# neonbjb/tortoise-tts

Hardware: NVIDIA H100
Metric: audio-seconds/sec at preset='standard' (higher is better)
Workload: dtype bf16 tensor-core operands, fp32 accumulate/residual/norm/softmax/scheduler

## Files before the change

tortoise_tts_b200/csrc/common.cuh:

```cuda
#pragma once
#include <cuda_runtime.h>
#include <cuda_bf16.h>
#include <cuda.h>
#include <stdint.h>
#include <cstdlib>

#define TTB_DEVINL __device__ __forceinline__

namespace ttb {

void set_error(const char* fmt, ...);
int check_cuda(cudaError_t e, const char* what);
#define TTB_CHECK_LAUNCH(what)                                   \
  do {                                                           \
    cudaError_t _e = cudaGetLastError();                         \
    if (_e != cudaSuccess) return ttb::check_cuda(_e, what);     \
  } while (0)

TTB_DEVINL void pdl_wait() { asm volatile("griddepcontrol.wait;" ::: "memory"); }
TTB_DEVINL void pdl_launch_dependents() { asm volatile("griddepcontrol.launch_dependents;" ::: "memory"); }

inline bool pdl_enabled() {
  static int v = -1;
  if (v < 0) {
    const char* e = getenv("TTB_PDL");
    v = (e && e[0] == '0') ? 0 : 1;
  }
  return v == 1;
}

template <typename... KArgs, typename... Args>
inline cudaError_t launch_pdl(void (*kernel)(KArgs...), dim3 grid, dim3 block, size_t smem, cudaStream_t st, Args&&... args) {
  cudaLaunchConfig_t cfg = {};
  cfg.gridDim = grid;
  cfg.blockDim = block;
  cfg.dynamicSmemBytes = smem;
  cfg.stream = st;
  cudaLaunchAttribute at[1];
  if (pdl_enabled()) {
    at[0].id = cudaLaunchAttributeProgrammaticStreamSerialization;
    at[0].val.programmaticStreamSerializationAllowed = 1;
    cfg.attrs = at;
    cfg.numAttrs = 1;
  }
  return cudaLaunchKernelEx(&cfg, kernel, static_cast<KArgs>(args)...);
}

TTB_DEVINL float silu(float x) { return x / (1.0f + __expf(-x)); }
TTB_DEVINL float gelu_new(float x) {
  const float k = 0.7978845608028654f;
  float u = k * (x + 0.044715f * x * x * x);
  return 0.5f * x * (1.0f + tanhf(u));
}
TTB_DEVINL float gelu_erf(float x) { return 0.5f * x * (1.0f + erff(x * 0.7071067811865476f)); }
TTB_DEVINL float leaky(float x, float s) { return x > 0.f ? x : x * s; }

TTB_DEVINL float warp_sum(float v) {
#pragma unroll
  for (int o = 16; o > 0; o >>= 1) v += __shfl_xor_sync(0xffffffffu, v, o);
  return v;
}
TTB_DEVINL float warp_max(float v) {
#pragma unroll
  for (int o = 16; o > 0; o >>= 1) v = fmaxf(v, __shfl_xor_sync(0xffffffffu, v, o));
  return v;
}

TTB_DEVINL float block_sum(float v, float* red) {
  int lane = threadIdx.x & 31, w = threadIdx.x >> 5, nw = (blockDim.x + 31) >> 5;
  v = warp_sum(v);
  __syncthreads();
  if (lane == 0) red[w] = v;
  __syncthreads();
  float r = (lane < nw) ? red[lane] : 0.f;
  r = warp_sum(r);
  return r;
}
TTB_DEVINL float block_max(float v, float* red) {
  int lane = threadIdx.x & 31, w = threadIdx.x >> 5, nw = (blockDim.x + 31) >> 5;
  v = warp_max(v);
  __syncthreads();
  if (lane == 0) red[w] = v;
  __syncthreads();
  float r = (lane < nw) ? red[lane] : -INFINITY;
  r = warp_max(r);
  return r;
}

TTB_DEVINL uint32_t pack_bf16(float a, float b) {
  __nv_bfloat162 t = __floats2bfloat162_rn(a, b);
  return *reinterpret_cast<uint32_t*>(&t);
}
TTB_DEVINL float2 unpack_bf16(uint32_t u) {
  __nv_bfloat162 t = *reinterpret_cast<__nv_bfloat162*>(&u);
  return __bfloat1622float2(t);
}

TTB_DEVINL uint32_t smem_u32(const void* p) { return static_cast<uint32_t>(__cvta_generic_to_shared(p)); }

TTB_DEVINL unsigned long long global_timer_ns() {
  unsigned long long t;
  asm volatile("mov.u64 %0, %%globaltimer;" : "=l"(t));
  return t;
}
TTB_DEVINL unsigned long long sm_id() {
  uint32_t s;
  asm volatile("mov.u32 %0, %%smid;" : "=r"(s));
  return s;
}

TTB_DEVINL bool elect_one() {
  uint32_t pred = 0;
  asm volatile(
      "{\n\t.reg .pred P;\n\t.reg .b32 R;\n\t"
      "elect.sync R|P, 0xffffffff;\n\t"
      "selp.u32 %0, 1, 0, P;\n\t}\n"
      : "=r"(pred));
  return pred != 0;
}

TTB_DEVINL void mbar_init(uint64_t* bar, uint32_t count) {
  asm volatile("mbarrier.init.shared::cta.b64 [%0], %1;" ::"r"(smem_u32(bar)), "r"(count));
}
TTB_DEVINL void fence_barrier_init() { asm volatile("fence.mbarrier_init.release.cluster;" ::: "memory"); }
TTB_DEVINL void fence_proxy_async() { asm volatile("fence.proxy.async.shared::cta;" ::: "memory"); }
TTB_DEVINL void mbar_arrive_expect_tx(uint64_t* bar, uint32_t bytes) {
  asm volatile("mbarrier.arrive.expect_tx.shared::cta.b64 _, [%0], %1;" ::"r"(smem_u32(bar)), "r"(bytes) : "memory");
}
TTB_DEVINL void mbar_arrive(uint64_t* bar) {
  asm volatile("mbarrier.arrive.shared::cta.b64 _, [%0];" ::"r"(smem_u32(bar)) : "memory");
}
#ifndef TTB_MBAR_HINT_NS
#define TTB_MBAR_HINT_NS 20000
#endif
TTB_DEVINL void mbar_wait(uint64_t* bar, uint32_t parity) {
#if TTB_MBAR_HINT_NS > 0
  asm volatile(
      "{\n\t.reg .pred P1;\n\t"
      "WAIT_LOOP:\n\t"
      "mbarrier.try_wait.parity.shared::cta.b64 P1, [%0], %1, %2;\n\t"
      "@P1 bra DONE;\n\t"
      "bra WAIT_LOOP;\n\t"
      "DONE:\n\t}\n" ::"r"(smem_u32(bar)),
      "r"(parity), "r"((uint32_t)TTB_MBAR_HINT_NS)
      : "memory");
#else
  asm volatile(
      "{\n\t.reg .pred P1;\n\t"
      "WAIT_LOOP:\n\t"
      "mbarrier.try_wait.parity.shared::cta.b64 P1, [%0], %1;\n\t"
      "@P1 bra DONE;\n\t"
      "bra WAIT_LOOP;\n\t"
      "DONE:\n\t}\n" ::"r"(smem_u32(bar)),
      "r"(parity)
      : "memory");
#endif
}

TTB_DEVINL void tma_prefetch_desc(const CUtensorMap* m) {
  asm volatile("prefetch.tensormap [%0];" ::"l"(reinterpret_cast<uint64_t>(m)) : "memory");
}
TTB_DEVINL void tma_load_2d(void* smem_dst, const CUtensorMap* map, uint64_t* bar, int c0, int c1) {
  asm volatile(
      "cp.async.bulk.tensor.2d.shared::cluster.global.mbarrier::complete_tx::bytes [%0], [%1, {%3, %4}], [%2];"
      ::"r"(smem_u32(smem_dst)), "l"(reinterpret_cast<uint64_t>(map)), "r"(smem_u32(bar)), "r"(c0), "r"(c1)
      : "memory");
}
TTB_DEVINL void tma_load_3d(void* smem_dst, const CUtensorMap* map, uint64_t* bar, int c0, int c1, int c2) {
  asm volatile(
      "cp.async.bulk.tensor.3d.shared::cluster.global.mbarrier::complete_tx::bytes [%0], [%1, {%3, %4, %5}], [%2];"
      ::"r"(smem_u32(smem_dst)), "l"(reinterpret_cast<uint64_t>(map)), "r"(smem_u32(bar)), "r"(c0), "r"(c1), "r"(c2)
      : "memory");
}
TTB_DEVINL void tma_prefetch_l2_3d(const CUtensorMap* map, int c0, int c1, int c2) {
  asm volatile("cp.async.bulk.prefetch.tensor.3d.L2.global.tile [%0, {%1, %2, %3}];"
               ::"l"(reinterpret_cast<uint64_t>(map)), "r"(c0), "r"(c1), "r"(c2)
               : "memory");
}

TTB_DEVINL void wgmma_fence() { asm volatile("wgmma.fence.sync.aligned;" ::: "memory"); }
TTB_DEVINL void wgmma_commit() { asm volatile("wgmma.commit_group.sync.aligned;" ::: "memory"); }
template <int N>
TTB_DEVINL void wgmma_wait() { asm volatile("wgmma.wait_group.sync.aligned %0;" ::"n"(N) : "memory"); }
TTB_DEVINL void named_barrier(int id, int nthreads) { asm volatile("bar.sync %0, %1;" ::"r"(id), "r"(nthreads) : "memory"); }

TTB_DEVINL uint64_t wgmma_desc_kmajor_sw128(uint32_t smem_addr) {
  uint64_t d = 0;
  d |= (uint64_t)((smem_addr & 0x3FFFF) >> 4);
  d |= (uint64_t)1 << 16;
  d |= (uint64_t)(1024 >> 4) << 32;
  d |= (uint64_t)1 << 62;
  return d;
}
TTB_DEVINL uint64_t wgmma_desc_mnmajor_sw128(uint32_t smem_addr, uint32_t lbo_bytes) {
  uint64_t d = 0;
  d |= (uint64_t)((smem_addr & 0x3FFFF) >> 4);
  d |= (uint64_t)((lbo_bytes >> 4) & 0x3FFF) << 16;
  d |= (uint64_t)(1024 >> 4) << 32;
  d |= (uint64_t)1 << 62;
  return d;
}

TTB_DEVINL void wgmma_m64n16k16_bf16_ss(float* d, uint64_t desc_a, uint64_t desc_b, uint32_t scale_d) {
  asm volatile(
      "{\n\t.reg .pred p;\n\tsetp.ne.b32 p, %10, 0;\n\t"
      "wgmma.mma_async.sync.aligned.m64n16k16.f32.bf16.bf16 {%0, %1, %2, %3, %4, %5, %6, %7}, %8, %9, p, 1, 1, 0, 0;\n\t}\n"
      : "+f"(d[0]), "+f"(d[1]), "+f"(d[2]), "+f"(d[3]), "+f"(d[4]), "+f"(d[5]), "+f"(d[6]), "+f"(d[7])
      : "l"(desc_a), "l"(desc_b), "r"(scale_d));
}
TTB_DEVINL void wgmma_m64n32k16_bf16_ss(float* d, uint64_t desc_a, uint64_t desc_b, uint32_t scale_d) {
  asm volatile(
      "{\n\t.reg .pred p;\n\tsetp.ne.b32 p, %18, 0;\n\t"
      "wgmma.mma_async.sync.aligned.m64n32k16.f32.bf16.bf16 {%0, %1, %2, %3, %4, %5, %6, %7, %8, %9, %10, %11, %12, %13, %14, %15}, %16, %17, p, 1, 1, 0, 0;\n\t}\n"
      : "+f"(d[0]), "+f"(d[1]), "+f"(d[2]), "+f"(d[3]), "+f"(d[4]), "+f"(d[5]), "+f"(d[6]), "+f"(d[7]), "+f"(d[8]), "+f"(d[9]), "+f"(d[10]), "+f"(d[11]), "+f"(d[12]), "+f"(d[13]), "+f"(d[14]), "+f"(d[15])
      : "l"(desc_a), "l"(desc_b), "r"(scale_d));
}
TTB_DEVINL void wgmma_m64n64k16_bf16_ss(float* d, uint64_t desc_a, uint64_t desc_b, uint32_t scale_d) {
  asm volatile(
      "{\n\t.reg .pred p;\n\tsetp.ne.b32 p, %34, 0;\n\t"
      "wgmma.mma_async.sync.aligned.m64n64k16.f32.bf16.bf16 {%0, %1, %2, %3, %4, %5, %6, %7, %8, %9, %10, %11, %12, %13, %14, %15, %16, %17, %18, %19, %20, %21, %22, %23, %24, %25, %26, %27, %28, %29, %30, %31}, %32, %33, p, 1, 1, 0, 0;\n\t}\n"
      : "+f"(d[0]), "+f"(d[1]), "+f"(d[2]), "+f"(d[3]), "+f"(d[4]), "+f"(d[5]), "+f"(d[6]), "+f"(d[7]), "+f"(d[8]), "+f"(d[9]), "+f"(d[10]), "+f"(d[11]), "+f"(d[12]), "+f"(d[13]), "+f"(d[14]), "+f"(d[15]), "+f"(d[16]), "+f"(d[17]), "+f"(d[18]), "+f"(d[19]), "+f"(d[20]), "+f"(d[21]), "+f"(d[22]), "+f"(d[23]), "+f"(d[24]), "+f"(d[25]), "+f"(d[26]), "+f"(d[27]), "+f"(d[28]), "+f"(d[29]), "+f"(d[30]), "+f"(d[31])
      : "l"(desc_a), "l"(desc_b), "r"(scale_d));
}
TTB_DEVINL void wgmma_m64n256k16_bf16_ss(float* d, uint64_t desc_a, uint64_t desc_b, uint32_t scale_d) {
  asm volatile(
      "{\n\t.reg .pred p;\n\tsetp.ne.b32 p, %130, 0;\n\t"
      "wgmma.mma_async.sync.aligned.m64n256k16.f32.bf16.bf16 {%0, %1, %2, %3, %4, %5, %6, %7, %8, %9, %10, %11, %12, %13, %14, %15, %16, %17, %18, %19, %20, %21, %22, %23, %24, %25, %26, %27, %28, %29, %30, %31, %32, %33, %34, %35, %36, %37, %38, %39, %40, %41, %42, %43, %44, %45, %46, %47, %48, %49, %50, %51, %52, %53, %54, %55, %56, %57, %58, %59, %60, %61, %62, %63, %64, %65, %66, %67, %68, %69, %70, %71, %72, %73, %74, %75, %76, %77, %78, %79, %80, %81, %82, %83, %84, %85, %86, %87, %88, %89, %90, %91, %92, %93, %94, %95, %96, %97, %98, %99, %100, %101, %102, %103, %104, %105, %106, %107, %108, %109, %110, %111, %112, %113, %114, %115, %116, %117, %118, %119, %120, %121, %122, %123, %124, %125, %126, %127}, %128, %129, p, 1, 1, 0, 0;\n\t}\n"
      : "+f"(d[0]), "+f"(d[1]), "+f"(d[2]), "+f"(d[3]), "+f"(d[4]), "+f"(d[5]), "+f"(d[6]), "+f"(d[7]), "+f"(d[8]), "+f"(d[9]), "+f"(d[10]), "+f"(d[11]), "+f"(d[12]), "+f"(d[13]), "+f"(d[14]), "+f"(d[15]), "+f"(d[16]), "+f"(d[17]), "+f"(d[18]), "+f"(d[19]), "+f"(d[20]), "+f"(d[21]), "+f"(d[22]), "+f"(d[23]), "+f"(d[24]), "+f"(d[25]), "+f"(d[26]), "+f"(d[27]), "+f"(d[28]), "+f"(d[29]), "+f"(d[30]), "+f"(d[31]), "+f"(d[32]), "+f"(d[33]), "+f"(d[34]), "+f"(d[35]), "+f"(d[36]), "+f"(d[37]), "+f"(d[38]), "+f"(d[39]), "+f"(d[40]), "+f"(d[41]), "+f"(d[42]), "+f"(d[43]), "+f"(d[44]), "+f"(d[45]), "+f"(d[46]), "+f"(d[47]), "+f"(d[48]), "+f"(d[49]), "+f"(d[50]), "+f"(d[51]), "+f"(d[52]), "+f"(d[53]), "+f"(d[54]), "+f"(d[55]), "+f"(d[56]), "+f"(d[57]), "+f"(d[58]), "+f"(d[59]), "+f"(d[60]), "+f"(d[61]), "+f"(d[62]), "+f"(d[63]), "+f"(d[64]), "+f"(d[65]), "+f"(d[66]), "+f"(d[67]), "+f"(d[68]), "+f"(d[69]), "+f"(d[70]), "+f"(d[71]), "+f"(d[72]), "+f"(d[73]), "+f"(d[74]), "+f"(d[75]), "+f"(d[76]), "+f"(d[77]), "+f"(d[78]), "+f"(d[79]), "+f"(d[80]), "+f"(d[81]), "+f"(d[82]), "+f"(d[83]), "+f"(d[84]), "+f"(d[85]), "+f"(d[86]), "+f"(d[87]), "+f"(d[88]), "+f"(d[89]), "+f"(d[90]), "+f"(d[91]), "+f"(d[92]), "+f"(d[93]), "+f"(d[94]), "+f"(d[95]), "+f"(d[96]), "+f"(d[97]), "+f"(d[98]), "+f"(d[99]), "+f"(d[100]), "+f"(d[101]), "+f"(d[102]), "+f"(d[103]), "+f"(d[104]), "+f"(d[105]), "+f"(d[106]), "+f"(d[107]), "+f"(d[108]), "+f"(d[109]), "+f"(d[110]), "+f"(d[111]), "+f"(d[112]), "+f"(d[113]), "+f"(d[114]), "+f"(d[115]), "+f"(d[116]), "+f"(d[117]), "+f"(d[118]), "+f"(d[119]), "+f"(d[120]), "+f"(d[121]), "+f"(d[122]), "+f"(d[123]), "+f"(d[124]), "+f"(d[125]), "+f"(d[126]), "+f"(d[127])
      : "l"(desc_a), "l"(desc_b), "r"(scale_d));
}
template <int TNSPB>
TTB_DEVINL void wgmma_m64n64k16_bf16_rs(float* d, const uint32_t* a, uint64_t desc_b, uint32_t scale_d) {
  asm volatile(
      "{\n\t.reg .pred p;\n\tsetp.ne.b32 p, %37, 0;\n\t"
      "wgmma.mma_async.sync.aligned.m64n64k16.f32.bf16.bf16 {%0, %1, %2, %3, %4, %5, %6, %7, %8, %9, %10, %11, %12, %13, %14, %15, %16, %17, %18, %19, %20, %21, %22, %23, %24, %25, %26, %27, %28, %29, %30, %31}, {%32, %33, %34, %35}, %36, p, 1, 1, %38;\n\t}\n"
      : "+f"(d[0]), "+f"(d[1]), "+f"(d[2]), "+f"(d[3]), "+f"(d[4]), "+f"(d[5]), "+f"(d[6]), "+f"(d[7]), "+f"(d[8]), "+f"(d[9]), "+f"(d[10]), "+f"(d[11]), "+f"(d[12]), "+f"(d[13]), "+f"(d[14]), "+f"(d[15]), "+f"(d[16]), "+f"(d[17]), "+f"(d[18]), "+f"(d[19]), "+f"(d[20]), "+f"(d[21]), "+f"(d[22]), "+f"(d[23]), "+f"(d[24]), "+f"(d[25]), "+f"(d[26]), "+f"(d[27]), "+f"(d[28]), "+f"(d[29]), "+f"(d[30]), "+f"(d[31])
      : "r"(a[0]), "r"(a[1]), "r"(a[2]), "r"(a[3]), "l"(desc_b), "r"(scale_d), "n"(TNSPB));
}

template <int BN>
TTB_DEVINL void gemm_mma_kblock(float* acc, uint32_t sa, uint32_t sb, bool first) {
  wgmma_fence();
#pragma unroll
  for (int k = 0; k < 4; ++k) {
    const uint64_t da = wgmma_desc_kmajor_sw128(sa + k * 32);
    const uint32_t sc = (first && k == 0) ? 0u : 1u;
    if constexpr (BN == 32) {
      wgmma_m64n32k16_bf16_ss(acc, da, wgmma_desc_kmajor_sw128(sb + k * 32), sc);
    } else {
#pragma unroll
      for (int nb = 0; nb < BN / 64; ++nb)
        wgmma_m64n64k16_bf16_ss(acc + nb * 32, da, wgmma_desc_kmajor_sw128(sb + nb * 8192 + k * 32), sc);
    }
  }
  wgmma_commit();
}

TTB_DEVINL void gemm_mma_kblock_n256(float* acc, uint32_t sa, uint32_t sb, bool first) {
  wgmma_fence();
#pragma unroll
  for (int k = 0; k < 4; ++k)
    wgmma_m64n256k16_bf16_ss(acc, wgmma_desc_kmajor_sw128(sa + k * 32), wgmma_desc_kmajor_sw128(sb + k * 32),
                             (first && k == 0) ? 0u : 1u);
  wgmma_commit();
}

template <int R>
TTB_DEVINL void setmaxnreg_dec() { asm volatile("setmaxnreg.dec.sync.aligned.u32 %0;" ::"n"(R)); }
template <int R>
TTB_DEVINL void setmaxnreg_inc() { asm volatile("setmaxnreg.inc.sync.aligned.u32 %0;" ::"n"(R)); }


}
```

tortoise_tts_b200/csrc/flash_attn.cu:

```cuda
#include <type_traits>

#include "common.cuh"
#include "ttb_internal.h"

namespace ttb {

constexpr int FA_BM = 128;
constexpr int FA_BN = 64;
constexpr int FA_CONSUMERS = 256;
constexpr int FA_PRODUCER_WARP = 8;
constexpr int FA_THREADS = FA_CONSUMERS + 32;
constexpr int FA_STAGES = 2;

struct FaSmem {
  static constexpr int Q_BYTES = FA_BM * 64 * 2;
  static constexpr int K_BYTES = FA_BN * 64 * 2;
  static constexpr int V_BYTES = FA_BN * 64 * 2;
  static constexpr int Q_OFF = 0;
  static constexpr int KV_OFF = Q_BYTES;
  static constexpr int BIAS_OFF = KV_OFF + FA_STAGES * (K_BYTES + V_BYTES);
  static constexpr int BAR_OFF = BIAS_OFF + 192 * 4;
  static constexpr int TOTAL = BAR_OFF + 16 * 8 + 1024;
};

__global__ void __launch_bounds__(FA_THREADS, 2)
flash_attn_tc_kernel(const __grid_constant__ CUtensorMap map_q, const __grid_constant__ CUtensorMap map_k,
                     const __grid_constant__ CUtensorMap map_v, TtbAttnArgs a) {
  extern __shared__ uint8_t smem_raw[];
  uint8_t* smem = reinterpret_cast<uint8_t*>((reinterpret_cast<uintptr_t>(smem_raw) + 1023) & ~uintptr_t(1023));
  uint64_t* bars = reinterpret_cast<uint64_t*>(smem + FaSmem::BAR_OFF);
  uint64_t* q_full = bars + 0;
  uint64_t* kv_full = bars + 1;
  uint64_t* kv_empty = bars + 1 + FA_STAGES;
  float* sbias = reinterpret_cast<float*>(smem + FaSmem::BIAS_OFF);

  const int warp = threadIdx.x >> 5, lane = threadIdx.x & 31;
  const int q0 = blockIdx.x * FA_BM, h = blockIdx.y, seq = blockIdx.z;
  const int Tq = a.T;
  const int T = a.Tk > 0 ? a.Tk : a.T;
  const int kv_end = a.causal ? min(T, q0 + FA_BM) : T;
  const int kc0 = a.kv_headmajor ? 0 : a.k_off + h * 64;
  const int vc0 = a.kv_headmajor ? 0 : a.v_off + h * 64;
  const int kvc2 = a.kv_headmajor ? h : seq;
  const int ntiles = (kv_end + FA_BN - 1) / FA_BN;

  if (warp == FA_PRODUCER_WARP && lane == 0) {
    tma_prefetch_desc(&map_q);
    tma_prefetch_desc(&map_k);
    tma_prefetch_desc(&map_v);
    mbar_init(q_full, 1);
    for (int s = 0; s < FA_STAGES; ++s) { mbar_init(&kv_full[s], 1); mbar_init(&kv_empty[s], 2); }
    fence_barrier_init();
  }
  __syncthreads();
  pdl_wait();

  if (warp == FA_PRODUCER_WARP) {
    if (lane == 0) {
      mbar_arrive_expect_tx(q_full, FaSmem::Q_BYTES);
      tma_load_3d(smem + FaSmem::Q_OFF, &map_q, q_full, h * 64, q0, seq);
      int stage = 0; uint32_t phase = 0;
      for (int j = 0; j < ntiles; ++j) {
        mbar_wait(&kv_empty[stage], phase ^ 1);
        uint8_t* sk = smem + FaSmem::KV_OFF + stage * (FaSmem::K_BYTES + FaSmem::V_BYTES);
        uint8_t* sv = sk + FaSmem::K_BYTES;
        mbar_arrive_expect_tx(&kv_full[stage], FaSmem::K_BYTES + FaSmem::V_BYTES);
        tma_load_3d(sk, &map_k, &kv_full[stage], kc0, j * FA_BN, kvc2);
        tma_load_3d(sv, &map_v, &kv_full[stage], vc0, j * FA_BN, kvc2);
        if (++stage == FA_STAGES) { stage = 0; phase ^= 1; }
      }
    }
    __syncwarp();
  } else {
    const int wg = warp >> 2;
    const int g = lane >> 2, t = lane & 3;
    const int row0 = wg * 64 + (warp & 3) * 16 + g;
    const float sl2 = a.scale * 1.4426950408889634f;
    const float* bias_h = a.bias ? a.bias + (long long)h * (2 * T - 1) + (T - 1) : nullptr;
    float m[2] = {-INFINITY, -INFINITY}, l[2] = {0.f, 0.f};
    float o[32];
#pragma unroll
    for (int i = 0; i < 32; ++i) o[i] = 0.f;
    const uint32_t sq = smem_u32(smem + FaSmem::Q_OFF) + wg * (64 * 128);
    mbar_wait(q_full, 0);
    int stage = 0; uint32_t phase = 0;
    for (int j = 0; j < ntiles; ++j) {
      const int k0 = j * FA_BN;
      const bool nomask = (k0 + FA_BN <= T) && (!a.causal || k0 + FA_BN - 1 <= q0);
      bool cbias_ok = (bias_h == nullptr);
      float cb = 0.f;
      if (bias_h && a.bias_sat > 0) {
        if (k0 - q0 + (FA_BN - 1) <= -a.bias_sat) { cbias_ok = true; cb = __ldg(bias_h - (T - 1)) * 1.4426950408889634f; }
        else if (k0 - q0 - (FA_BM - 1) >= a.bias_sat) { cbias_ok = true; cb = __ldg(bias_h + (T - 1)) * 1.4426950408889634f; }
      }
      const bool fast = nomask && cbias_ok;
      if (bias_h && !fast) {
        named_barrier(1, FA_CONSUMERS);
        for (int i = threadIdx.x; i < 191; i += FA_CONSUMERS) {
          const int rel = k0 - q0 - 127 + i;
          sbias[i] = (rel > -T && rel < T) ? __ldg(bias_h + rel) * 1.4426950408889634f : 0.f;
        }
        named_barrier(1, FA_CONSUMERS);
      }
      mbar_wait(&kv_full[stage], phase);
      const uint32_t sk = smem_u32(smem + FaSmem::KV_OFF + stage * (FaSmem::K_BYTES + FaSmem::V_BYTES));
      const uint32_t sv = sk + FaSmem::K_BYTES;
      float s[32];
      wgmma_fence();
#pragma unroll
      for (int k = 0; k < 4; ++k)
        wgmma_m64n64k16_bf16_ss(s, wgmma_desc_kmajor_sw128(sq + k * 32), wgmma_desc_kmajor_sw128(sk + k * 32), k != 0);
      wgmma_commit();
      wgmma_wait<0>();
      float mx[2] = {-INFINITY, -INFINITY};
      if (fast) {
#pragma unroll
        for (int i = 0; i < 32; ++i) mx[(i >> 1) & 1] = fmaxf(mx[(i >> 1) & 1], s[i]);
        mx[0] = fmaf(mx[0], sl2, cb);
        mx[1] = fmaf(mx[1], sl2, cb);
      } else {
#pragma unroll
        for (int i = 0; i < 32; ++i) {
          const int hh = (i >> 1) & 1;
          const int row = row0 + 8 * hh;
          const int c = 8 * (i >> 2) + 2 * t + (i & 1);
          const int klim = min(T - k0, a.causal ? (q0 + row - k0 + 1) : FA_BN);
          float v = s[i] * sl2;
          if (bias_h) v += sbias[c - row + 127];
          v = (c < klim) ? v : -INFINITY;
          s[i] = v;
          mx[hh] = fmaxf(mx[hh], v);
        }
      }
      float corr[2], cm[2];
#pragma unroll
      for (int hh = 0; hh < 2; ++hh) {
        mx[hh] = fmaxf(mx[hh], __shfl_xor_sync(0xffffffffu, mx[hh], 1));
        mx[hh] = fmaxf(mx[hh], __shfl_xor_sync(0xffffffffu, mx[hh], 2));
        const bool grow = mx[hh] > m[hh] + 8.0f;
        const float m_new = grow ? mx[hh] : m[hh];
        corr[hh] = grow ? exp2f(m[hh] - m_new) : 1.0f;
        m[hh] = m_new;
        const float m_use = (m_new == -INFINITY) ? 0.f : m_new;
        cm[hh] = fast ? cb - m_use : -m_use;
      }
      float psum[2] = {0.f, 0.f};
      uint32_t pa[16];
#pragma unroll
      for (int i = 0; i < 32; i += 2) {
        const int hh = (i >> 1) & 1;
        const float p0 = fast ? exp2f(fmaf(s[i], sl2, cm[hh])) : exp2f(s[i] + cm[hh]);
        const float p1 = fast ? exp2f(fmaf(s[i + 1], sl2, cm[hh])) : exp2f(s[i + 1] + cm[hh]);
        psum[hh] += p0 + p1;
        pa[i >> 1] = pack_bf16(p0, p1);
      }
#pragma unroll
      for (int hh = 0; hh < 2; ++hh) l[hh] = l[hh] * corr[hh] + psum[hh];
#pragma unroll
      for (int i = 0; i < 32; ++i) o[i] *= corr[(i >> 1) & 1];
      wgmma_fence();
#pragma unroll
      for (int k = 0; k < 4; ++k)
        wgmma_m64n64k16_bf16_rs<1>(o, pa + 4 * k, wgmma_desc_mnmajor_sw128(sv + k * 2048, 0), 1u);
      wgmma_commit();
      wgmma_wait<0>();
      if ((threadIdx.x & 127) == 0) mbar_arrive(&kv_empty[stage]);
      if (++stage == FA_STAGES) { stage = 0; phase ^= 1; }
    }
#pragma unroll
    for (int hh = 0; hh < 2; ++hh) {
      l[hh] += __shfl_xor_sync(0xffffffffu, l[hh], 1);
      l[hh] += __shfl_xor_sync(0xffffffffu, l[hh], 2);
      const int qi = q0 + row0 + 8 * hh;
      if (qi >= Tq) continue;
      const float inv = 1.0f / l[hh];
      if (a.lse) {
        float* op = a.out_f32 + ((long long)seq * Tq + qi) * a.ldo + h * 64 + 2 * t;
#pragma unroll
        for (int nb = 0; nb < 8; ++nb)
          *reinterpret_cast<float2*>(op + 8 * nb) = make_float2(o[4 * nb + 2 * hh] * inv, o[4 * nb + 2 * hh + 1] * inv);
        if (t == 0) a.lse[((long long)seq * Tq + qi) * a.H + h] = m[hh] + log2f(l[hh]);
      } else {
        __nv_bfloat16* op = reinterpret_cast<__nv_bfloat16*>(a.out) + ((long long)seq * Tq + qi) * a.ldo + h * 64 + 2 * t;
#pragma unroll
        for (int nb = 0; nb < 8; ++nb)
          *reinterpret_cast<uint32_t*>(op + 8 * nb) = pack_bf16(o[4 * nb + 2 * hh] * inv, o[4 * nb + 2 * hh + 1] * inv);
      }
    }
  }
  pdl_launch_dependents();
}

static int g_fa_mode = -1;

bool flash_attention_supported(const TtbAttnArgs& a) {
  if (g_fa_mode < 0) {
    const char* e = getenv("TTB_ATTN_IMPL");
    g_fa_mode = (e && strcmp(e, "simt") == 0) ? 0 : 1;
  }
  if (!g_fa_mode) return false;
  if (a.kv || a.lse) return true;
  return a.T >= 64 && (a.ld % 8) == 0;
}

int flash_attention_launch(const TtbAttnArgs& a, cudaStream_t st) {
  CUtensorMap mq, mk, mv;
  if (get_tensor_map_bf16(&mq, a.qkv, (uint64_t)a.ld, (uint64_t)a.T, (uint64_t)a.nseq, (uint64_t)a.ld,
                          (uint64_t)a.T * a.ld, 64, FA_BM)) return -1;
  if (a.kv_headmajor) {
    if (!a.kv || !a.kv_v || a.Tk <= 0 || a.causal || a.bias) { set_error("flash attention: bad head-major KV arguments"); return -1; }
    if (get_tensor_map_bf16(&mk, a.kv, 64, (uint64_t)a.Tk, (uint64_t)a.H, 64, (uint64_t)a.Tk * 64, 64, FA_BN)) return -1;
    if (get_tensor_map_bf16(&mv, a.kv_v, 64, (uint64_t)a.Tk, (uint64_t)a.H, 64, (uint64_t)a.Tk * 64, 64, FA_BN)) return -1;
  } else {
    if (a.Tk > 0 && a.Tk != a.T) { set_error("flash attention: Tk != T needs the head-major KV form"); return -1; }
    if (get_tensor_map_bf16(&mk, a.qkv, (uint64_t)a.ld, (uint64_t)a.T, (uint64_t)a.nseq, (uint64_t)a.ld,
                            (uint64_t)a.T * a.ld, 64, FA_BN)) return -1;
    mv = mk;
  }
  if (a.lse && !a.out_f32) { set_error("flash attention: lse output needs out_f32"); return -1; }
  static bool attr = false;
  if (!attr) {
    cudaError_t r = cudaFuncSetAttribute(flash_attn_tc_kernel, cudaFuncAttributeMaxDynamicSharedMemorySize, FaSmem::TOTAL);
    if (r != cudaSuccess) return check_cuda(r, "cudaFuncSetAttribute(flash_attn)");
    attr = true;
  }
  dim3 grid((a.T + FA_BM - 1) / FA_BM, a.H, a.nseq);
  const cudaError_t le = launch_pdl(flash_attn_tc_kernel, grid, dim3(FA_THREADS), (size_t)FaSmem::TOTAL, st, mq, mk, mv, a);
  if (le != cudaSuccess) return check_cuda(le, "flash_attn_tc_kernel launch");
  TTB_CHECK_LAUNCH("flash_attn_tc_kernel");
  return 0;
}

}
```

Measured before the change: 7.404.

## Restructure flash attention into FA3-style pingpong warpgroups with intra-warpgroup overlap

The flash attention kernel now uses a full producer warpgroup with register reallocation (setmaxnreg) and two consumer warpgroups that alternate tensor-core issue through named barriers. The QK^T of the next tile overlaps with softmax of the current one while P·V runs, and the KV pipeline deepens from 2 to 4 stages. The whole relative-position bias row is preloaded into shared memory once per block instead of per tile, and the O rescale is skipped when no correction occurred. In exchange, occupancy drops to one block per SM, shared memory grows substantially, and biased attention is now limited to T <= 8192.

```diff
diff --git a/tortoise_tts_b200/csrc/common.cuh b/tortoise_tts_b200/csrc/common.cuh
--- a/tortoise_tts_b200/csrc/common.cuh
+++ b/tortoise_tts_b200/csrc/common.cuh
@@ -183,6 +183,7 @@
 template <int N>
 TTB_DEVINL void wgmma_wait() { asm volatile("wgmma.wait_group.sync.aligned %0;" ::"n"(N) : "memory"); }
 TTB_DEVINL void named_barrier(int id, int nthreads) { asm volatile("bar.sync %0, %1;" ::"r"(id), "r"(nthreads) : "memory"); }
+TTB_DEVINL void named_barrier_arrive(int id, int nthreads) { asm volatile("bar.arrive %0, %1;" ::"r"(id), "r"(nthreads) : "memory"); }
 
 TTB_DEVINL uint64_t wgmma_desc_kmajor_sw128(uint32_t smem_addr) {
   uint64_t d = 0;
diff --git a/tortoise_tts_b200/csrc/flash_attn.cu b/tortoise_tts_b200/csrc/flash_attn.cu
--- a/tortoise_tts_b200/csrc/flash_attn.cu
+++ b/tortoise_tts_b200/csrc/flash_attn.cu
@@ -7,10 +7,10 @@
 
 constexpr int FA_BM = 128;
 constexpr int FA_BN = 64;
-constexpr int FA_CONSUMERS = 256;
-constexpr int FA_PRODUCER_WARP = 8;
-constexpr int FA_THREADS = FA_CONSUMERS + 32;
-constexpr int FA_STAGES = 2;
+constexpr int FA_THREADS = 384;
+constexpr int FA_STAGES = 4;
+constexpr int FA_BIAS_MAX_T = 8192;
+constexpr float FA_LOG2E = 1.4426950408889634f;
 
 struct FaSmem {
   static constexpr int Q_BYTES = FA_BM * 64 * 2;
@@ -19,11 +19,62 @@
   static constexpr int Q_OFF = 0;
   static constexpr int KV_OFF = Q_BYTES;
   static constexpr int BIAS_OFF = KV_OFF + FA_STAGES * (K_BYTES + V_BYTES);
-  static constexpr int BAR_OFF = BIAS_OFF + 192 * 4;
+  static constexpr int BIAS_FLOATS = FA_BIAS_MAX_T + FA_BM;
+  static constexpr int BAR_OFF = BIAS_OFF + BIAS_FLOATS * 4;
   static constexpr int TOTAL = BAR_OFF + 16 * 8 + 1024;
+  static_assert(TOTAL <= 227 * 1024, "flash attention shared memory");
 };
 
-__global__ void __launch_bounds__(FA_THREADS, 2)
+template <bool FAST>
+TTB_DEVINL void fa_softmax_tile(float (&s)[32], float (&m)[2], float (&l)[2], float (&corr)[2], float sl2, float cb,
+                                const float* sbias, int k0, int klim_max, int causal_lim, int row, int t) {
+  float mx[2] = {-INFINITY, -INFINITY};
+  if (FAST) {
+#pragma unroll
+    for (int i = 0; i < 32; ++i) mx[(i >> 1) & 1] = fmaxf(mx[(i >> 1) & 1], s[i]);
+    mx[0] = fmaf(mx[0], sl2, cb);
+    mx[1] = fmaf(mx[1], sl2, cb);
+  } else {
+#pragma unroll
+    for (int i = 0; i < 32; ++i) {
+      const int hh = (i >> 1) & 1;
+      const int r = row + 8 * hh;
+      const int c = 8 * (i >> 2) + 2 * t + (i & 1);
+      const int klim = min(klim_max, causal_lim + r);
+      float v = s[i] * sl2;
+      if (sbias) v += sbias[k0 + c - r + (FA_BM - 1)];
+      v = (c < klim) ? v : -INFINITY;
+      s[i] = v;
+      mx[hh] = fmaxf(mx[hh], v);
+    }
+  }
+  float cm[2];
+#pragma unroll
+  for (int hh = 0; hh < 2; ++hh) {
+    mx[hh] = fmaxf(mx[hh], __shfl_xor_sync(0xffffffffu, mx[hh], 1));
+    mx[hh] = fmaxf(mx[hh], __shfl_xor_sync(0xffffffffu, mx[hh], 2));
+    const bool grow = mx[hh] > m[hh] + 8.0f;
+    const float m_new = grow ? mx[hh] : m[hh];
+    corr[hh] = grow ? exp2f(m[hh] - m_new) : 1.0f;
+    m[hh] = m_new;
+    const float m_use = (m_new == -INFINITY) ? 0.f : m_new;
+    cm[hh] = FAST ? cb - m_use : -m_use;
+  }
+  float psum[2] = {0.f, 0.f};
+#pragma unroll
+  for (int i = 0; i < 32; i += 2) {
+    const int hh = (i >> 1) & 1;
+    const float p0 = FAST ? exp2f(fmaf(s[i], sl2, cm[hh])) : exp2f(s[i] + cm[hh]);
+    const float p1 = FAST ? exp2f(fmaf(s[i + 1], sl2, cm[hh])) : exp2f(s[i + 1] + cm[hh]);
+    psum[hh] += p0 + p1;
+    s[i] = p0;
+    s[i + 1] = p1;
+  }
+#pragma unroll
+  for (int hh = 0; hh < 2; ++hh) l[hh] = l[hh] * corr[hh] + psum[hh];
+}
+
+__global__ void __launch_bounds__(FA_THREADS, 1)
 flash_attn_tc_kernel(const __grid_constant__ CUtensorMap map_q, const __grid_constant__ CUtensorMap map_k,
                      const __grid_constant__ CUtensorMap map_v, TtbAttnArgs a) {
   extern __shared__ uint8_t smem_raw[];
@@ -44,7 +95,7 @@
   const int kvc2 = a.kv_headmajor ? h : seq;
   const int ntiles = (kv_end + FA_BN - 1) / FA_BN;
 
-  if (warp == FA_PRODUCER_WARP && lane == 0) {
+  if (threadIdx.x == 0) {
     tma_prefetch_desc(&map_q);
     tma_prefetch_desc(&map_k);
     tma_prefetch_desc(&map_v);
@@ -55,8 +106,9 @@
   __syncthreads();
   pdl_wait();
 
-  if (warp == FA_PRODUCER_WARP) {
-    if (lane == 0) {
+  if (warp < 4) {
+    setmaxnreg_dec<40>();
+    if (threadIdx.x == 0) {
       mbar_arrive_expect_tx(q_full, FaSmem::Q_BYTES);
       tma_load_3d(smem + FaSmem::Q_OFF, &map_q, q_full, h * 64, q0, seq);
       int stage = 0; uint32_t phase = 0;
@@ -72,101 +124,103 @@
     }
     __syncwarp();
   } else {
-    const int wg = warp >> 2;
+    setmaxnreg_inc<232>();
+    const int wg = (warp >> 2) - 1;
     const int g = lane >> 2, t = lane & 3;
     const int row0 = wg * 64 + (warp & 3) * 16 + g;
-    const float sl2 = a.scale * 1.4426950408889634f;
+    const float sl2 = a.scale * FA_LOG2E;
     const float* bias_h = a.bias ? a.bias + (long long)h * (2 * T - 1) + (T - 1) : nullptr;
-    float m[2] = {-INFINITY, -INFINITY}, l[2] = {0.f, 0.f};
-    float o[32];
-#pragma unroll
-    for (int i = 0; i < 32; ++i) o[i] = 0.f;
-    const uint32_t sq = smem_u32(smem + FaSmem::Q_OFF) + wg * (64 * 128);
-    mbar_wait(q_full, 0);
-    int stage = 0; uint32_t phase = 0;
-    for (int j = 0; j < ntiles; ++j) {
-      const int k0 = j * FA_BN;
+    if (bias_h) {
+      for (int i = threadIdx.x - 128; i < ntiles * FA_BN + FA_BM - 1; i += 256) {
+        const int rel = i - q0 - (FA_BM - 1);
+        sbias[i] = (rel > -T && rel < T) ? __ldg(bias_h + rel) * FA_LOG2E : 0.f;
+      }
+      named_barrier(1, 256);
+    }
+    const int my_turn = 2 + wg, next_turn = 2 + (wg ^ 1);
+    if (wg == 1) named_barrier_arrive(next_turn, 256);
+
+    auto softmax = [&](float (&s)[32], int k0, float (&m)[2], float (&l)[2], float (&corr)[2]) {
       const bool nomask = (k0 + FA_BN <= T) && (!a.causal || k0 + FA_BN - 1 <= q0);
       bool cbias_ok = (bias_h == nullptr);
       float cb = 0.f;
       if (bias_h && a.bias_sat > 0) {
-        if (k0 - q0 + (FA_BN - 1) <= -a.bias_sat) { cbias_ok = true; cb = __ldg(bias_h - (T - 1)) * 1.4426950408889634f; }
-        else if (k0 - q0 - (FA_BM - 1) >= a.bias_sat) { cbias_ok = true; cb = __ldg(bias_h + (T - 1)) * 1.4426950408889634f; }
-      }
-      const bool fast = nomask && cbias_ok;
-      if (bias_h && !fast) {
-        named_barrier(1, FA_CONSUMERS);
-        for (int i = threadIdx.x; i < 191; i += FA_CONSUMERS) {
-          const int rel = k0 - q0 - 127 + i;
-          sbias[i] = (rel > -T && rel < T) ? __ldg(bias_h + rel) * 1.4426950408889634f : 0.f;
-        }
-        named_barrier(1, FA_CONSUMERS);
-      }
-      mbar_wait(&kv_full[stage], phase);
-      const uint32_t sk = smem_u32(smem + FaSmem::KV_OFF + stage * (FaSmem::K_BYTES + FaSmem::V_BYTES));
-      const uint32_t sv = sk + FaSmem::K_BYTES;
-      float s[32];
-      wgmma_fence();
+        if (k0 - q0 + (FA_BN - 1) <= -a.bias_sat) { cbias_ok = true; cb = __ldg(bias_h - (T - 1)) * FA_LOG2E; }
+        else if (k0 - q0 - (FA_BM - 1) >= a.bias_sat) { cbias_ok = true; cb = __ldg(bias_h + (T - 1)) * FA_LOG2E; }
+      }
+      if (nomask && cbias_ok) {
+        fa_softmax_tile<true>(s, m, l, corr, sl2, cb, nullptr, k0, 0, 0, 0, t);
+      } else {
+        fa_softmax_tile<false>(s, m, l, corr, sl2, 0.f, bias_h ? sbias : nullptr, k0, min(T - k0, FA_BN),
+                               a.causal ? q0 + 1 - k0 : FA_BN, row0, t);
+      }
+    };
+
+    float m[2] = {-INFINITY, -INFINITY}, l[2] = {0.f, 0.f}, corr[2];
+    float o[32], s[32];
+    uint32_t pa[16];
+#pragma unroll
+    for (int i = 0; i < 32; ++i) o[i] = 0.f;
+    const uint32_t sq = smem_u32(smem + FaSmem::Q_OFF) + wg * (64 * 128);
+    auto kv_addr = [&](int st) { return smem_u32(smem + FaSmem::KV_OFF + st * (FaSmem::K_BYTES + FaSmem::V_BYTES)); };
+    auto issue_s = [&](uint32_t sk) {
 #pragma unroll
       for (int k = 0; k < 4; ++k)
         wgmma_m64n64k16_bf16_ss(s, wgmma_desc_kmajor_sw128(sq + k * 32), wgmma_desc_kmajor_sw128(sk + k * 32), k != 0);
       wgmma_commit();
-      wgmma_wait<0>();
-      float mx[2] = {-INFINITY, -INFINITY};
-      if (fast) {
-#pragma unroll
-        for (int i = 0; i < 32; ++i) mx[(i >> 1) & 1] = fmaxf(mx[(i >> 1) & 1], s[i]);
-        mx[0] = fmaf(mx[0], sl2, cb);
-        mx[1] = fmaf(mx[1], sl2, cb);
-      } else {
-#pragma unroll
-        for (int i = 0; i < 32; ++i) {
-          const int hh = (i >> 1) & 1;
-          const int row = row0 + 8 * hh;
-          const int c = 8 * (i >> 2) + 2 * t + (i & 1);
-          const int klim = min(T - k0, a.causal ? (q0 + row - k0 + 1) : FA_BN);
-          float v = s[i] * sl2;
-          if (bias_h) v += sbias[c - row + 127];
-          v = (c < klim) ? v : -INFINITY;
-          s[i] = v;
-          mx[hh] = fmaxf(mx[hh], v);
-        }
-      }
-      float corr[2], cm[2];
-#pragma unroll
-      for (int hh = 0; hh < 2; ++hh) {
-        mx[hh] = fmaxf(mx[hh], __shfl_xor_sync(0xffffffffu, mx[hh], 1));
-        mx[hh] = fmaxf(mx[hh], __shfl_xor_sync(0xffffffffu, mx[hh], 2));
-        const bool grow = mx[hh] > m[hh] + 8.0f;
-        const float m_new = grow ? mx[hh] : m[hh];
-        corr[hh] = grow ? exp2f(m[hh] - m_new) : 1.0f;
-        m[hh] = m_new;
-        const float m_use = (m_new == -INFINITY) ? 0.f : m_new;
-        cm[hh] = fast ? cb - m_use : -m_use;
-      }
-      float psum[2] = {0.f, 0.f};
-      uint32_t pa[16];
-#pragma unroll
-      for (int i = 0; i < 32; i += 2) {
-        const int hh = (i >> 1) & 1;
-        const float p0 = fast ? exp2f(fmaf(s[i], sl2, cm[hh])) : exp2f(s[i] + cm[hh]);
-        const float p1 = fast ? exp2f(fmaf(s[i + 1], sl2, cm[hh])) : exp2f(s[i + 1] + cm[hh]);
-        psum[hh] += p0 + p1;
-        pa[i >> 1] = pack_bf16(p0, p1);
-      }
-#pragma unroll
-      for (int hh = 0; hh < 2; ++hh) l[hh] = l[hh] * corr[hh] + psum[hh];
-#pragma unroll
-      for (int i = 0; i < 32; ++i) o[i] *= corr[(i >> 1) & 1];
-      wgmma_fence();
+    };
+
+    auto pack_p = [&]() {
+#pragma unroll
+      for (int i = 0; i < 16; ++i) pa[i] = pack_bf16(s[2 * i], s[2 * i + 1]);
+    };
+    mbar_wait(q_full, 0);
+    mbar_wait(&kv_full[0], 0);
+    named_barrier(my_turn, 256);
+    wgmma_fence();
+    issue_s(kv_addr(0));
+    named_barrier_arrive(next_turn, 256);
+    wgmma_wait<0>();
+    softmax(s, 0, m, l, corr);
+    pack_p();
+
+    auto issue_pv = [&](uint32_t sv) {
 #pragma unroll
       for (int k = 0; k < 4; ++k)
         wgmma_m64n64k16_bf16_rs<1>(o, pa + 4 * k, wgmma_desc_mnmajor_sw128(sv + k * 2048, 0), 1u);
       wgmma_commit();
+    };
+    auto rescale_o = [&]() {
+      if (__any_sync(0xffffffffu, corr[0] != 1.0f || corr[1] != 1.0f)) {
+#pragma unroll
+        for (int i = 0; i < 32; ++i) o[i] *= corr[(i >> 1) & 1];
+      }
+    };
+
+    int stage = 0; uint32_t phase = 0;
+    for (int j = 1; j < ntiles; ++j) {
+      const int nstage = stage + 1 == FA_STAGES ? 0 : stage + 1;
+      const uint32_t nphase = nstage == 0 ? phase ^ 1 : phase;
+      mbar_wait(&kv_full[nstage], nphase);
+      rescale_o();
+      named_barrier(my_turn, 256);
+      wgmma_fence();
+      issue_s(kv_addr(nstage));
+      issue_pv(kv_addr(stage) + FaSmem::K_BYTES);
+      named_barrier_arrive(next_turn, 256);
+      wgmma_wait<1>();
+      softmax(s, j * FA_BN, m, l, corr);
       wgmma_wait<0>();
       if ((threadIdx.x & 127) == 0) mbar_arrive(&kv_empty[stage]);
-      if (++stage == FA_STAGES) { stage = 0; phase ^= 1; }
-    }
+      pack_p();
+      stage = nstage; phase = nphase;
+    }
+    rescale_o();
+    named_barrier(my_turn, 256);
+    wgmma_fence();
+    issue_pv(kv_addr(stage) + FaSmem::K_BYTES);
+    if (wg == 0) named_barrier_arrive(next_turn, 256);
+    wgmma_wait<0>();
 #pragma unroll
     for (int hh = 0; hh < 2; ++hh) {
       l[hh] += __shfl_xor_sync(0xffffffffu, l[hh], 1);
@@ -218,6 +272,10 @@
     mv = mk;
   }
   if (a.lse && !a.out_f32) { set_error("flash attention: lse output needs out_f32"); return -1; }
+  if (a.bias && a.T > FA_BIAS_MAX_T) {
+    set_error("flash attention: a bias table needs T <= %d (got %d)", FA_BIAS_MAX_T, a.T);
+    return -1;
+  }
   static bool attr = false;
   if (!attr) {
     cudaError_t r = cudaFuncSetAttribute(flash_attn_tc_kernel, cudaFuncAttributeMaxDynamicSharedMemorySize, FaSmem::TOTAL);
```

Measured after the change: 7.571 (median of 6 runs). 2.3% higher.
